# duongve13112002/DiffusionSpatialControl

Hardware: AMD Instinct MI355X
Metric: 512x512 images/sec, SD1.5 25-step DPM++2M Karras with region-biased cross-attention (higher is better)
Workload: dtype f16; 1 GPU; SD1.5 512x512, 25-step DPM++2M Karras, CFG 7.5, 2 region masks, 1 image(s) per generation, 2 generation(s) in flight per GPU; images_per_gpu=1, parallelism=dp1 (independent images, no per-step collective), hip_graph=True, outputs_finite=True, full=False

## Files before the change

diffusionspatialcontrol_amd/_lib.py:

```python
import ctypes
import os
import re

_HERE = os.path.dirname(os.path.abspath(__file__))
_LIB = None


class DscLibraryError(RuntimeError):
    pass


def lib_path():
    return os.environ.get("DSC_LIB_PATH") or os.path.join(_HERE, "libdsc_hip.so")


def header_path():
    return os.path.join(os.path.dirname(_HERE), "include", "dsc_hip.h")


def declared_symbols():
    txt = open(header_path()).read()
    txt = re.sub(r"/\*.*?\*/", "", txt, flags=re.S)
    return sorted(set(re.findall(r"\b(dsc_[a-z0-9_]+)\s*\(", txt)))

# ... 75 lines not shown
                                          ctypes.c_int, ctypes.c_int, _vp, ctypes.c_int, _vp, ctypes.c_float, ctypes.c_int, _vp]),
    "dsc_add_layernorm": (ctypes.c_int, [_vp] * 6 + [ctypes.c_int64, ctypes.c_int, ctypes.c_float, ctypes.c_int, _vp]),
    "dsc_geglu": (ctypes.c_int, [_vp, _vp, ctypes.c_int64, ctypes.c_int, ctypes.c_int, _vp]),
    "dsc_linear_splitk_workspace_bytes": (ctypes.c_size_t, [ctypes.c_int64, ctypes.c_int, ctypes.c_int, ctypes.c_int]),
    "dsc_linear_splitk_f16": (ctypes.c_int, [_vp] * 5 + [ctypes.c_int64, ctypes.c_int, ctypes.c_int] + [ctypes.c_int64] * 3 +
                              [ctypes.c_int, _vp, ctypes.c_size_t, ctypes.c_int, _vp]),
    "dsc_conv3x3_gn_rows": (ctypes.c_int, [ctypes.c_int] * 7),
    "dsc_conv3x3_gn_nhwc_f16": (ctypes.c_int, [_vp] * 4 + [ctypes.c_int64, _vp, _vp] + [ctypes.c_int] * 5 + [ctypes.c_int64] * 3 +
                                [ctypes.c_int, _vp, ctypes.c_int, ctypes.c_int, _vp]),
    "dsc_linear_gn_rows": (ctypes.c_int, [ctypes.c_int64, ctypes.c_int, ctypes.c_int, ctypes.c_int, ctypes.c_int]),
    "dsc_linear_gn_f16": (ctypes.c_int, [_vp] * 5 + [ctypes.c_int64, ctypes.c_int, ctypes.c_int] + [ctypes.c_int64] * 3 +
                          [ctypes.c_int, _vp, ctypes.c_int, ctypes.c_int, _vp]),
    "dsc_groupnorm_apply_nhwc": (ctypes.c_int, [_vp] * 5 + [ctypes.c_int] * 5 + [ctypes.c_float, ctypes.c_int, ctypes.c_int, _vp]),
    "dsc_softmax_rows_f16": (ctypes.c_int, [_vp, _vp, ctypes.c_int64, ctypes.c_int, ctypes.c_int64, ctypes.c_int64, ctypes.c_float,
                                            ctypes.c_int, _vp]),
    "dsc_latent_resample_noise": (ctypes.c_int, [_vp] * 3 + [ctypes.c_int] * 6 + [_vp] * 4 + [ctypes.c_float, _vp]),
}


def load_library():
    global _LIB
    if _LIB is not None:
        return _LIB
    import torch
    path = lib_path()
    if not os.path.exists(path):
        raise DscLibraryError(
            f"{path} not found: build it with `python -c 'import __graft_entry__ as g; g.build()'` "
            "(hipcc --offload-arch=gfx950).  There is no CPU fallback for the HIP hot path.")
    try:
# ... 33 lines not shown
```

diffusionspatialcontrol_amd/csrc/conv3x3.hip:

```cpp
#include "dsc_common.h"
#include "dsc_hip.h"
#include "gn_partials.h"
#include <type_traits>

extern int g_dsc_tuning_profile;

namespace {

constexpr int BM = 128, BN = 64, BK = 64, T = 256;
constexpr int kBStageBytes = BN * BK * 2;
constexpr int kAPiecesMax = 25;
constexpr int kABytes = kAPiecesMax * 1024;
constexpr int kRingOff = 0;
constexpr int a_off(int S) { return S * kBStageBytes; }
constexpr int pad_off(int S) { return a_off(S) + 2 * kABytes; }
constexpr int lds_bytes(int S) { return pad_off(S) + 1024; }
constexpr int a_bytes(int NT, int TW) { return NT == 4 && TW == 16 ? 23 * 1024 : kABytes; }
constexpr int lds_bytes_up2x(int TW) { return a_off(4) + 2 * a_bytes(4, TW) + 1024; }
constexpr int kEpiStride = BN + 4;
constexpr unsigned kOob = 0x80000000u;

struct ConvParams {
    const half_t* x; const half_t* w; const half_t* bias; const half_t* res; half_t* out; float* ws;
    int B, H, W, Cin, Cout;
// ... 485 lines not shown
        9ll * Cin * Cout >= (1ll << 30)) return 0;
    return plan(B, H, W, Cin, Cout, 0, &p) ? 1 : 0;
}

extern "C" size_t dsc_conv3x3_workspace_bytes(int B, int H, int W, int Cin, int Cout, int splits) {
    ConvParams p{};
    if (B <= 0 || H <= 0 || W <= 0 || !plan(B, H, W, Cin, Cout, splits, &p)) return 0;
    return p.splits > 1 ? (size_t)p.splits * p.npix * Cout * sizeof(float) : 0;
}

namespace {
struct GnArgs { const void* add; int64_t add_ld; float* part; int groups; };
int conv_impl(const void* x, const void* w, const void* bias, const void* residual, void* out,
              int B, int H, int W, int Cin, int Cout, int64_t ldx, int64_t ldr, int64_t ldo,
              int resample, int out_nchw, int splits, int dtype, void* workspace, size_t workspace_bytes, void* stream,
              const GnArgs* gn);
}

extern "C" int dsc_conv3x3_nhwc_f16(const void* x, const void* w, const void* bias, const void* residual, void* out,
                                    int B, int H, int W, int Cin, int Cout, int64_t ldx, int64_t ldr, int64_t ldo,
                                    int resample, int out_nchw, int splits, int dtype, void* workspace,
                                    size_t workspace_bytes, void* stream) {
    return conv_impl(x, w, bias, residual, out, B, H, W, Cin, Cout, ldx, ldr, ldo, resample, out_nchw, splits, dtype, workspace,
                     workspace_bytes, stream, nullptr);
}

extern "C" int dsc_conv3x3_gn_rows(int B, int H, int W, int Cin, int Cout, int groups, int resample) {
    ConvParams p{};
    const int Hc = H, Wc = W;
    if (B <= 0 || H <= 0 || W <= 0 || groups <= 0 || Cout % BN != 0 || Cout % groups != 0 || Cout / groups > 64 || Cout / groups < 2) return 0;
    if (resample == DSC_CONV_STRIDE2 || resample == DSC_CONV_STRIDE2_PAD_BR) return 0;
// ... 5 lines not shown
extern "C" int dsc_conv3x3_gn_nhwc_f16(const void* x, const void* w, const void* bias, const void* add, int64_t add_ld,
                                       const void* residual, void* out, int B, int H, int W, int Cin, int Cout, int64_t ldx,
                                       int64_t ldr, int64_t ldo, int resample, float* gn_part, int groups, int dtype, void* stream) {
    if (!gn_part || groups <= 0) return DSC_ERR_BAD_ARG;
    if (!dsc_conv3x3_gn_rows(B, H, W, Cin, Cout, groups, resample)) return DSC_ERR_UNSUPPORTED;
    if (add && (add_ld < Cout || add_ld % 8 != 0 || (reinterpret_cast<uintptr_t>(add) & 15))) return DSC_ERR_UNSUPPORTED;
    if (reinterpret_cast<uintptr_t>(gn_part) & 7) return DSC_ERR_UNSUPPORTED;
    const GnArgs gn{add, add_ld, gn_part, groups};
    return conv_impl(x, w, bias, residual, out, B, H, W, Cin, Cout, ldx, ldr, ldo, resample, 0, 1, dtype, nullptr, 0, stream, &gn);
}

namespace {
int conv_impl(const void* x, const void* w, const void* bias, const void* residual, void* out,
              int B, int H, int W, int Cin, int Cout, int64_t ldx, int64_t ldr, int64_t ldo,
              int resample, int out_nchw, int splits, int dtype, void* workspace, size_t workspace_bytes, void* stream,
              const GnArgs* gn) {
    if (!x || !w || !out || B <= 0 || H <= 0 || W <= 0 || Cin <= 0 || Cout <= 0) return DSC_ERR_BAD_ARG;
    if (dtype != DSC_F16) return DSC_ERR_UNSUPPORTED;
    if (ldx < Cin || (!out_nchw && ldo < Cout) || (residual && ldr < Cout)) return DSC_ERR_BAD_ARG;
    if (ldx % 8 != 0 || (Cout % 8 == 0 && !out_nchw && ldo % 8 != 0) || (residual && Cout % 8 == 0 && ldr % 8 != 0)) return DSC_ERR_UNSUPPORTED;
    if (!al16(x) || !al16(w) || !al16(out) || (bias && !al16(bias)) || (residual && !al16(residual))) return DSC_ERR_UNSUPPORTED;
    if ((long long)B * H * W * (ldx > ldo ? ldx : ldo) >= (1ll << 30) || 9ll * Cin * Cout >= (1ll << 30)) return DSC_ERR_UNSUPPORTED;
    ConvParams p{};
    const int tw = plan(B, H, W, Cin, Cout, splits, &p);
    if (!tw) return DSC_ERR_UNSUPPORTED;
    p.x = static_cast<const half_t*>(x); p.w = static_cast<const half_t*>(w);
    p.bias = static_cast<const half_t*>(bias); p.res = static_cast<const half_t*>(residual);
    p.out = static_cast<half_t*>(out); p.ws = static_cast<float*>(workspace);
    p.ldx = ldx; p.ldr = ldr; p.ldo = ldo;
    p.stamps = g_conv_stamps;
    if (gn) {
        p.add = static_cast<const half_t*>(gn->add); p.add_ld = gn->add_ld;
        p.gn_part = gn->part; p.gn_G = gn->groups; p.gn_cpg = Cout / gn->groups;
    }
    p.order = g_conv_order >= 0 ? g_conv_order : (p.npix >= 2ll * Cout ? 1 : 0);
    if (resample < 0 || resample > 4 || ((resample == DSC_CONV_STRIDE2 || resample == DSC_CONV_STRIDE2_PAD_BR) && out_nchw)) return DSC_ERR_UNSUPPORTED;
    if (resample == DSC_CONV_STRIDE2_PAD_BR && ((H | W) & 1)) return DSC_ERR_UNSUPPORTED;
    p.up = resample == DSC_CONV_UPSAMPLE2X || resample == DSC_CONV_UPSAMPLE_CEIL ? 1 : 0;
    p.sh = resample == DSC_CONV_UPSAMPLE_CEIL ? (H + 1) / 2 : H / 2; p.sw = resample == DSC_CONV_UPSAMPLE_CEIL ? (W + 1) / 2 : W / 2;
    p.sub2 = resample == DSC_CONV_STRIDE2 ? 1 : (resample == DSC_CONV_STRIDE2_PAD_BR ? 2 : 0);
// ... 22 lines not shown
    const dim3 grid(((total + 7) / 8) * 8), block(T);
    int ring = g_conv_ring;
    if (ring != 3 && ring != 9) ring = (total <= 256 && g_dsc_tuning_profile == DSC_TUNE_LATENCY) ? 9 : 3;
    const bool loaders = ring == 9 && (g_conv_loaders == 2 || (g_conv_loaders == 1 && tw == 16));
    const dim3 block8(T + 256);
    if (tw == 16) {
        if (loaders) DSC_LAUNCH((conv3x3_kernel<16, 9, 4>), grid, block8, (size_t)lds_bytes(9), st, p);
        else if (ring == 9) DSC_LAUNCH((conv3x3_kernel<16, 9>), grid, block, (size_t)lds_bytes(9), st, p);
        else DSC_LAUNCH((conv3x3_kernel<16, 3>), grid, block, (size_t)lds_bytes(3), st, p);
    } else {
        if (loaders) DSC_LAUNCH((conv3x3_kernel<8, 9, 4>), grid, block8, (size_t)lds_bytes(9), st, p);
        else if (ring == 9) DSC_LAUNCH((conv3x3_kernel<8, 9>), grid, block, (size_t)lds_bytes(9), st, p);
        else DSC_LAUNCH((conv3x3_kernel<8, 3>), grid, block, (size_t)lds_bytes(3), st, p);
    }
    if (hipGetLastError() != hipSuccess) return DSC_ERR_LAUNCH;
    if (p.splits > 1) {
        const long long n = p.onpix * (Cout / 8);
        p.fd_cv = make_fastdiv(Cout / 8, n + 256);
        DSC_LAUNCH(conv3x3_reduce, dim3((unsigned)((n + 255) / 256)), dim3(256), 0, st, p);
        if (hipGetLastError() != hipSuccess) return DSC_ERR_LAUNCH;
    }
    return DSC_OK;
}
}


namespace {

__global__ __launch_bounds__(256) void conv3x3_up2x_pack_kernel(const half_t* __restrict__ w, half_t* __restrict__ packed, int Cin, int Cout) {
    const int cv = Cin >> 3;
    const long long idx = (long long)blockIdx.x * 256 + threadIdx.x;
    if (idx >= 16ll * Cout * cv) return;
    const int c = (int)(idx % cv) * 8;
    const int tap = (int)(idx / cv) & 3;
    const long long pn = idx / cv / 4;
    const int n = (int)(pn % Cout), phase = (int)(pn / Cout);
    const int py = phase >> 1, px = phase & 1, a = tap >> 1, b = tap & 1;
    const int dy0 = py + a == 0 ? 0 : (py + a == 2 ? 2 : 1 - py), dy1 = py + a == 1 ? dy0 + 1 : dy0;
// ... 87 lines not shown
```

diffusionspatialcontrol_amd/csrc/gemm.hip:

```cpp
#include "dsc_common.h"
#include "dsc_hip.h"
#include "gn_partials.h"

extern int g_dsc_tuning_profile;

namespace {

constexpr int BN = 64, BK = 64, T = 256;
constexpr int kBHalves = BN * BK;
constexpr int a_halves(int bm) { return bm * BK; }
constexpr int stage_halves(int bm, int nt = 1) { return bm * BK + nt * kBHalves; }
constexpr int epi_stride(int nt = 1) { return nt * BN + 4; }
constexpr int kEpiStride = epi_stride(1);

struct GemmParams {
    const half_t* x; const half_t* w; const half_t* bias; const half_t* res; half_t* out;
    int M, N, K;
    long long ldx, ldr, ldo;
    const float* ln_in;
    const float* ln_c;
    float* ln_out;
    int ln_nb; float ln_inv_c, ln_eps;
    half_t* kv; int kv_C, kv_H, kv_d, kv_L, kv_B;
    int xcd_remap, total;
// ... 322 lines not shown
    const long long m = fdiv(idx, fd_cv);
    const int n = (idx - (int)m * cv) * 8;
    float acc[8] = {0, 0, 0, 0, 0, 0, 0, 0};
    for (int k = 0; k < splits; ++k) {
        const float* src = ws + ((long long)k * M + m) * N + n;
        const f4x_t a = *reinterpret_cast<const f4x_t*>(src), b = *reinterpret_cast<const f4x_t*>(src + 4);
#pragma unroll
        for (int j = 0; j < 4; ++j) { acc[j] += a[j]; acc[4 + j] += b[j]; }
    }
    h8_t bv = {0, 0, 0, 0, 0, 0, 0, 0}, rv = {0, 0, 0, 0, 0, 0, 0, 0};
    if (bias) bv = *reinterpret_cast<const h8_t*>(bias + n);
    if (res) rv = *reinterpret_cast<const h8_t*>(res + m * ldr + n);
    h8_t o;
#pragma unroll
    for (int j = 0; j < 8; ++j) o[j] = (half_t)(acc[j] + (float)bv[j] + (float)rv[j]);
    *reinterpret_cast<h8_t*>(out + m * ldo + n) = o;
}

bool al16(const void* q) { return (reinterpret_cast<uintptr_t>(q) & 15) == 0; }

long long* g_gemm_stamps = nullptr;
int g_gemm_stages = 0;
int g_gemm_bm = 0;
int g_gemm_loaders = 0;
int g_gemm_xcd = 0;
int g_gemm_wide_min = 512;
int g_gemm_ntstore = 0;
int g_gemm_nt = 0;

}
// ... 213 lines not shown
    if (splits <= 1) return dsc_linear_f16(x, w, bias, residual, out, M, N, K, ldx, ldr, ldo, 0, dtype, stream);
    if (residual && (ldr >> 32) != 0) return DSC_ERR_UNSUPPORTED;
    const size_t need = (size_t)splits * M * N * sizeof(float);
    if (!workspace || workspace_bytes < need || !al16(workspace)) return DSC_ERR_WORKSPACE;
    if ((bias && !al16(bias)) || (residual && (!al16(residual) || ldr % 8 != 0)) || ldo % 8 != 0 || !al16(out)) return DSC_ERR_UNSUPPORTED;
    const int rc = linear_impl(x, w, nullptr, nullptr, out, M, N, K, ldx, 0, ldo, 0, nullptr, 0, nullptr, 0.f, nullptr, dtype, stream,
                               nullptr, 0, 0, splits, static_cast<float*>(workspace));
    if (rc != DSC_OK) return rc;
    const long long n8 = M * (N / 8);
    if (n8 >= (1ll << 30)) return DSC_ERR_UNSUPPORTED;
    DSC_LAUNCH(gemm_splitk_reduce, dim3((unsigned)((n8 + 255) / 256)), dim3(256), 0, static_cast<hipStream_t>(stream),
               static_cast<const float*>(workspace), static_cast<const half_t*>(bias), static_cast<const half_t*>(residual),
               static_cast<half_t*>(out), (long long)M, N, splits, (long long)ldr, (long long)ldo, make_fastdiv(N / 8, n8 + 256));
    return hipGetLastError() == hipSuccess ? DSC_OK : DSC_ERR_LAUNCH;
}
```

diffusionspatialcontrol_amd/csrc/groupnorm_nhwc.hip:

```cpp
#include "dsc_common.h"
#include "dsc_hip.h"

namespace {

constexpr int kMaxT = 512;

struct GnN {
    const half_t* x; half_t* y; const half_t* gamma; const half_t* beta; const half_t* add;
    double* partials;
    float* stats;
    int B, HW, C, G, cpg, cv, k, nchunk, rows;
    int anchunk, arows;
    int inline_stats;
    int scv, nslab, sk;
    long long add_stride;
    float eps; int silu;
    const half_t* x2; half_t* cat; int C1;
    const float* fpart; int fPT;
    FastDiv fd_G, fd_anchunk, fd_cv, fd_cpg, fd_vpp, fd_nslab, fd_nchunk, fd_scv;
};

__device__ __forceinline__ h8_t gn_load(const GnN& p, int b, int pix, int c) {
    const long long bp = (long long)b * p.HW + pix;
    if (!p.x2) return *reinterpret_cast<const h8_t*>(p.x + bp * p.C + c);
    const h8_t v = c < p.C1 ? *reinterpret_cast<const h8_t*>(p.x + bp * p.C1 + c)
                            : *reinterpret_cast<const h8_t*>(p.x2 + bp * (p.C - p.C1) + (c - p.C1));
    *reinterpret_cast<h8_t*>(p.cat + bp * p.C + c) = v;
    return v;
}

__global__ __launch_bounds__(kMaxT) void gn_nhwc_stats(GnN p) {
    extern __shared__ __attribute__((aligned(16))) char smem[];
    const int bc = fdiv(blockIdx.x, p.fd_nslab), slab = blockIdx.x - bc * p.nslab;
    const int b = fdiv(bc, p.fd_nchunk), chunk = bc - b * p.nchunk;
    const int v0 = slab * p.scv;
// ... 232 lines not shown
    for (int i = 0; i < kSmallVec; ++i) {
        const int idx = threadIdx.x + 256 * i;
        if (idx < nvec) {
            const int pix = fdiv(idx, p.fd_vpp), j8 = idx - pix * vpp;
            const h8_t ga = gav[i], be = bev[i];
            h8_t o;
#pragma unroll
            for (int j = 0; j < 8; ++j) {
                float f = (v[i][j] - mean) * rstd * (float)ga[j] + (float)be[j];
                if (p.silu) f = silu_f(f);
                o[j] = (half_t)f;
            }
            *reinterpret_cast<h8_t*>(p.y + base + (long long)pix * p.C + j8 * 8) = o;
        }
    }
}

struct GnBundle { int gb, nvec, npl; };

template <int T, int NV>
__global__ __launch_bounds__(T) void gn_nhwc_bundle(GnN p, GnBundle q) {
    extern __shared__ __attribute__((aligned(16))) char smem[];
    float* S = reinterpret_cast<float*>(smem);
    __shared__ float gstat[8];
    const int nb = p.G / q.gb;
    const int b = blockIdx.x / nb, bun = blockIdx.x % nb;
    const int cw = q.nvec * 8;
    const int t = threadIdx.x;
    const bool active = t < q.nvec * q.npl;
    const int v = t % q.nvec, lp = t / q.nvec;
// ... 280 lines not shown
                                        void* stream) {
    if (!x || !y || !gamma || !beta || !gn_part || part_rows <= 0 || B <= 0 || C <= 0 || hw <= 0 || groups <= 0) return DSC_ERR_BAD_ARG;
    if (dtype != DSC_F16) return DSC_ERR_UNSUPPORTED;
    GnN p{};
    p.B = B; p.C = C; p.HW = hw; p.G = groups;
    if (!plan(p) || p.cpg > 64 || C % 64 != 0) return DSC_ERR_UNSUPPORTED;
    if (!al16(x) || !al16(y) || !al16(gamma) || !al16(beta) || !al16(gn_part)) return DSC_ERR_UNSUPPORTED;
    p.x = static_cast<const half_t*>(x); p.y = static_cast<half_t*>(y);
    p.gamma = static_cast<const half_t*>(gamma); p.beta = static_cast<const half_t*>(beta);
    p.eps = eps; p.silu = apply_silu;
    p.fpart = gn_part; p.fPT = part_rows; p.inline_stats = 1;
    gn_fastdivs(p);
    DSC_LAUNCH(gn_nhwc_apply, dim3(B * p.anchunk), dim3(p.cv * p.k), 0, static_cast<hipStream_t>(stream), p);
    return hipGetLastError() == hipSuccess ? DSC_OK : DSC_ERR_LAUNCH;
}
```

diffusionspatialcontrol_amd/modules/u_net_condition_modify.py:

```python
import inspect
import math
from dataclasses import dataclass, field
from typing import Any, Dict, Optional, Tuple

import torch
import torch.nn as nn
import torch.nn.functional as F

from .. import ops
from .attention_modify import AttnProcessor, AttnProcessor2_0


class ImageProjection(nn.Module):

    def __init__(self, image_embed_dim=768, cross_attention_dim=768, num_image_text_embeds=32):
        super().__init__()
        self.num_image_text_embeds = num_image_text_embeds
        self.image_embeds = nn.Linear(image_embed_dim, num_image_text_embeds * cross_attention_dim)
        self.norm = nn.LayerNorm(cross_attention_dim)

    def forward(self, image_embeds):
        b = image_embeds.shape[0]
        return self.norm(self.image_embeds(image_embeds).reshape(b, self.num_image_text_embeds, -1))

# ... 460 lines not shown
        return _derived(self, "tb", (self.time_emb_proj.bias, self.conv1.bias),
                        lambda: (self.time_emb_proj.bias + self.conv1.bias).contiguous())

    def forward(self, x, temb_act, temb_add=None):
        if isinstance(x, tuple):
            h, x = self.norm1.of_cat(*x)
        else:
            h = self.norm1(x)
        if temb_add is None:
            temb_add = F.linear(temb_act, self.time_emb_proj.weight, self.temb_bias())
        g = self.norm2.num_groups
        fuse = h.is_cuda and h.dtype == torch.float16 and h.shape[0] * h.shape[2] * h.shape[3] >= GN_FUSE_MIN_ROWS
        if fuse and ops.conv3x3_gn_rows(h, self.conv1.weight, g) > 0:
            h = self.norm2(ops.conv3x3_gn(h, self.conv1.weight, g, add=temb_add[:h.shape[0]]))
        else:
            h = self.norm2(_conv3x3(h, self.conv1.weight), add=temb_add)
        if self.conv_shortcut is None:
            if fuse and ops.conv3x3_gn_rows(h, self.conv2.weight, g) > 0:
                return ops.conv3x3_gn(h, self.conv2.weight, g, bias=self.conv2.bias, residual=x)
            return _conv3x3(h, self.conv2.weight, self.conv2.bias, residual=x)
        h = _conv3x3(h, self.conv2.weight)
        b = _derived(self, "sb", (self.conv_shortcut.bias, self.conv2.bias),
                     lambda: (self.conv_shortcut.bias + self.conv2.bias).contiguous())
        bsz, _, hh, ww = h.shape
        t, part = self.conv_shortcut.tokens(_tokens(x), bias=b, residual=_tokens(h), gn_groups=g)
        return _with_gn(_image(t, hh, ww), part)


class Downsample2D(nn.Module):
    def __init__(self, c):
        super().__init__()
        self.conv = nn.Conv2d(c, c, 3, stride=2, padding=1)

    def forward(self, x):
        if ops.conv3x3_supported(x, self.conv.weight):
            return ops.conv3x3(x, self.conv.weight, self.conv.bias, stride2_ceil=True)
        return self.conv(x)


# ... 301 lines not shown
```

diffusionspatialcontrol_amd/ops.py:

```python
import ctypes
import os

import numpy as np
import torch

from . import _lib

FLAG_REF_FP16_ROUNDING = 1
FLAG_BIAS_IS_FINAL = 2
FLAG_REUSE_STATS = 4
FLAG_ROWS_PADDED = 256
FLAG_SIGMA_PER_GROUP = 512
REGION_ROW_STRIDE = 100

def _stream_ptr(t):
    return ctypes.c_void_p(torch.cuda.current_stream(t.device).cuda_stream)


def _p(t):
    return ctypes.c_void_p(t.data_ptr()) if t is not None else None


def _i64x3(a, b, c):
    return (ctypes.c_int64 * 3)(a, b, c)
# ... 572 lines not shown
        part, cvec, eps = ln
        nb = part.shape[1]
        if part.shape[0] != M or part.dtype != torch.float32 or not part.is_contiguous() or cvec.numel() != 3 * C:
            raise ValueError("linear_qkv: statistics / cvec do not match the operands")
    rc = _lib.load_library().dsc_linear_qkv_f16(_p(x2), _p(weight), _p(bias), _p(q), _p(kv), M, C, K, x2.stride(0), C, heads, L,
                                                _p(part), nb, _p(cvec), float(eps), 0, _stream_ptr(x))
    _lib.check(rc, "dsc_linear_qkv_f16")
    return q.view(B, L, heads, d), kv[0].permute(0, 2, 1, 3), kv[1].permute(0, 2, 1, 3)


USE_SPLITK = os.environ.get("DSC_GEMM_SPLITK", "1") != "0"
SPLITK_MAX_ROWS = int(os.environ.get("DSC_SPLITK_MAX_ROWS", "512"))
SPLITK_MIN_K = int(os.environ.get("DSC_SPLITK_MIN_K", "1920"))


def linear_splitk(x2, weight, bias, r2, splits=0):
    lib = _lib.load_library()
    M, K = x2.shape
    N = weight.shape[0]
    out = torch.empty((M, N), dtype=x2.dtype, device=x2.device)
    nbytes = lib.dsc_linear_splitk_workspace_bytes(M, N, K, splits)
    ws = _workspace(x2.device, nbytes) if nbytes else None
    rc = lib.dsc_linear_splitk_f16(_p(x2), _p(weight), _p(bias), _p(r2), _p(out), M, N, K, x2.stride(0),
                                   r2.stride(0) if r2 is not None else 0, N, splits, _p(ws), ws.numel() * 8 if ws is not None else 0,
                                   0, _stream_ptr(x2))
    _lib.check(rc, "dsc_linear_splitk_f16")
    return out


def linear(x, weight, bias=None, residual=None, geglu=False, prefer_kernel=False):
# ... 9 lines not shown
    x2 = None
    if can:
        x2 = x.reshape(M, K)
        can = x2.stride(1) == 1 and x2.stride(0) % 8 == 0 and x2.data_ptr() % 16 == 0
    ldr = 0
    if residual is not None and residual.numel() != M * N:
        got = _residual_2d(residual, M, N) if can and not geglu else None
        if got is None or not (prefer_kernel or _gemm_rows_k_preferred(M, K, geglu)):
            residual = residual.reshape(-1, N).repeat(M // (residual.numel() // N), 1).reshape(*lead, N)
    if can and residual is not None:
        got = _residual_2d(residual, M, N)
        can = got is not None
        if can:
            r2, ldr = got
    ok = can and (prefer_kernel or _gemm_rows_k_preferred(M, K, geglu))
    if can and not ok and not geglu and USE_SPLITK and not USE_LIBRARY_GEMM and M <= SPLITK_MAX_ROWS and K >= SPLITK_MIN_K \
            and (bias is None or (bias.dtype == torch.float16 and bias.data_ptr() % 16 == 0)):
        return linear_splitk(x2, weight, bias, residual.reshape(M, N) if residual is not None else None).reshape(*lead, N)
    if not ok:
        if ((USE_LT_RESIDUAL if residual is not None else USE_LT_ALL) and x.dtype == torch.float16 and K % 8 == 0
                and N % 8 == 0 and M >= 8 and not (geglu and residual is not None)):
            xl = x.reshape(M, K)
            rl = residual.reshape(M, N) if residual is not None else None
            if (xl.stride(1) == 1 and xl.stride(0) % 8 == 0 and weight.is_contiguous() and weight.dtype == torch.float16
                    and (bias is None or bias.dtype == torch.float16)
                    and (rl is None or (rl.stride(1) == 1 and rl.stride(0) % 8 == 0))):
                out = torch.empty((M, N), dtype=x.dtype, device=x.device)
                rc = _lib.load_library().dsc_linear_lt_f16(_p(xl), _p(weight), _p(bias), _p(rl), _p(out), M, N, K,
                                                           xl.stride(0), rl.stride(0) if rl is not None else 0, N, 0,
                                                           _stream_ptr(x))
                if rc == 0:
                    out = out.reshape(*lead, N)
# ... 70 lines not shown
        out = torch.empty((B, Cout, oh, ow), dtype=x.dtype, device=x.device, memory_format=cl)
    ldr = 0
    if residual is not None:
        if residual.shape != out.shape:
            raise ValueError("conv3x3: residual must have the output's shape")
        if not residual.is_contiguous(memory_format=cl):
            residual = residual.contiguous(memory_format=cl)
        ldr = Cout
    nbytes = lib.dsc_conv3x3_workspace_bytes(B, H, W, Cin, Cout, splits)
    ws = _workspace(x.device, nbytes) if nbytes else None
    rc = lib.dsc_conv3x3_nhwc_f16(_p(x), _p(weight), _p(bias), _p(residual), _p(out), B, H, W, Cin, Cout, Cin, ldr, Cout,
                                  3 if stride2_pad_br else (2 if stride2 else (1 if upsample else (4 if size is not None else 0))), 1 if out_nchw else 0, splits, 0, _p(ws),
                                  ws.numel() * 8 if ws is not None else 0, _stream_ptr(x))
    _lib.check(rc, "dsc_conv3x3_nhwc_f16")
    return out


USE_UP2X_PHASES = os.environ.get("DSC_UP2X_PHASES", "1") != "0"


def conv3x3_up2x_pack(weight):
    _require_gpu(weight)
    if weight.dim() != 4 or tuple(weight.shape[2:]) != (3, 3) or weight.dtype != torch.float16:
        raise ValueError("conv3x3_up2x_pack: weight must be a [Cout, Cin, 3, 3] fp16 tensor")
    Cout, Cin = weight.shape[:2]
    if Cin % 64 != 0:
        raise ValueError("conv3x3_up2x_pack: Cin must be a multiple of 64")
    cl = torch.channels_last
    if not weight.is_contiguous(memory_format=cl):
        weight = weight.contiguous(memory_format=cl)
# ... 340 lines not shown
```

include/dsc_hip.h:

```cpp
#ifndef DSC_HIP_H
#define DSC_HIP_H

#include <stddef.h>
#include <stdint.h>

#ifdef __cplusplus
extern "C" {
#endif

#define DSC_OK                0
#define DSC_ERR_BAD_ARG      -1
#define DSC_ERR_UNSUPPORTED  -2
#define DSC_ERR_WORKSPACE    -3
#define DSC_ERR_LAUNCH       -4

#define DSC_F16 0
#define DSC_FLAG_REF_FP16_ROUNDING 1u
#define DSC_FLAG_REUSE_STATS       4u
#define DSC_FLAG_ROWS_PADDED     256u
#define DSC_FLAG_BIAS_IS_FINAL     2u
#define DSC_FLAG_SIGMA_PER_GROUP 512u

int dsc_abi_version(void);
const char* dsc_target_arch(void);
// ... 95 lines not shown
size_t dsc_groupnorm_workspace_bytes(int B, int C, int hw, int groups);
int dsc_groupnorm_silu(const void* x, void* y, const void* gamma, const void* beta,
                       int B, int C, int hw, int groups, float eps, int apply_silu, int dtype,
                       void* workspace, size_t workspace_bytes, void* stream);

size_t dsc_groupnorm_nhwc_workspace_bytes(int B, int C, int hw, int groups);
void dsc_debug_set_gn_mode(int mode);
int dsc_groupnorm_silu_nhwc(const void* x, void* y, const void* gamma, const void* beta,
                            const void* add, int64_t add_row_stride,
                            int B, int C, int hw, int groups, float eps, int apply_silu, int dtype,
                            void* workspace, size_t workspace_bytes, void* stream);
int dsc_groupnorm_silu_nhwc_cat(const void* x1, const void* x2, int C1, void* cat, void* y, const void* gamma,
                                const void* beta, const void* add, int64_t add_row_stride, int B, int C, int hw,
                                int groups, float eps, int apply_silu, int dtype, void* workspace, size_t workspace_bytes,
                                void* stream);

int dsc_add_bias_residual(const void* a, const void* b, const void* bias, void* out, int64_t rows, int C,
                          int dtype, void* stream);

int dsc_linear_f16(const void* x, const void* w, const void* bias, const void* residual, void* out,
                   int64_t M, int N, int K, int64_t ldx, int64_t ldr, int64_t ldo, int geglu, int dtype, void* stream);

#define DSC_CONV_UPSAMPLE2X 1
#define DSC_CONV_STRIDE2 2
#define DSC_CONV_STRIDE2_PAD_BR 3
#define DSC_CONV_UPSAMPLE_CEIL 4
int dsc_conv3x3_supported(int B, int H, int W, int Cin, int Cout);
void dsc_debug_set_conv_stamps(void* device_buffer);
void dsc_debug_set_conv_ring(int stages);
size_t dsc_conv3x3_workspace_bytes(int B, int H, int W, int Cin, int Cout, int splits);
int dsc_conv3x3_nhwc_f16(const void* x, const void* w, const void* bias, const void* residual, void* out,
                         int B, int H, int W, int Cin, int Cout, int64_t ldx, int64_t ldr, int64_t ldo,
                         int resample, int out_nchw, int splits, int dtype, void* workspace, size_t workspace_bytes,
                         void* stream);

int dsc_conv3x3_up2x_pack_f16(const void* w, void* packed, int Cin, int Cout, void* stream);
int dsc_conv3x3_up2x_supported(int B, int h, int w, int Cin, int Cout);
size_t dsc_conv3x3_up2x_workspace_bytes(int B, int h, int w, int Cin, int Cout, int splits);
int dsc_conv3x3_up2x_nhwc_f16(const void* x, const void* w_packed, const void* bias, void* out, int B, int h, int w,
                              int Cin, int Cout, int splits, void* workspace, size_t workspace_bytes, int64_t ldx,
                              int64_t ldo, int dtype, void* stream);

int dsc_linear_ln_f16(const void* x, const void* w, const void* bias, const void* residual, void* out,
                      int64_t M, int N, int K, int64_t ldx, int64_t ldr, int64_t ldo, int geglu,
                      const float* ln_in, int ln_nb, const float* ln_cvec, float ln_eps, float* ln_out,
                      int dtype, void* stream);
void dsc_debug_set_gemm_stages(int stages);
int dsc_linear_qkv_f16(const void* x, const void* w, const void* bias, void* q_out, void* kv_out,
                       int64_t M, int C, int K, int64_t ldx, int64_t ldq, int heads, int seq_len,
// ... 26 lines not shown
int dsc_conv3x3_gn_nhwc_f16(const void* x, const void* w, const void* bias, const void* add, int64_t add_ld,
                            const void* residual, void* out, int B, int H, int W, int Cin, int Cout, int64_t ldx,
                            int64_t ldr, int64_t ldo, int resample, float* gn_part, int groups, int dtype, void* stream);
int dsc_linear_gn_rows(int64_t M, int N, int K, int rows_per_image, int groups);
int dsc_linear_gn_f16(const void* x, const void* w, const void* bias, const void* residual, void* out,
                      int64_t M, int N, int K, int64_t ldx, int64_t ldr, int64_t ldo, int rows_per_image,
                      float* gn_part, int groups, int dtype, void* stream);
int dsc_groupnorm_apply_nhwc(const void* x, void* y, const void* gamma, const void* beta, const float* gn_part,
                             int part_rows, int B, int C, int hw, int groups, float eps, int apply_silu, int dtype,
                             void* stream);

size_t dsc_linear_splitk_workspace_bytes(int64_t M, int N, int K, int splits);
int dsc_linear_splitk_f16(const void* x, const void* w, const void* bias, const void* residual, void* out,
                          int64_t M, int N, int K, int64_t ldx, int64_t ldr, int64_t ldo, int splits,
                          void* workspace, size_t workspace_bytes, int dtype, void* stream);

int dsc_softmax_rows_f16(const void* scores, void* probs, int64_t rows, int n, int64_t ld_scores, int64_t ld_probs,
                         float scale, int dtype, void* stream);

int dsc_latent_resample_noise(const void* src, const void* noise, void* dst, int n, int C, int h, int w, int H, int W,
                              const int* idx_y, const float* w_y, const int* idx_x, const float* w_x,
                              float noise_scale_f16_value, void* stream);

#ifdef __cplusplus
}
#endif
#endif
```

Baseline: 11.90 images/s.

## Fold split-K conv partial-plane reduction into groupnorm and shortcut GEMM reduce

For small-resolution ResNet blocks where the 3x3 conv runs split-K, a new path skips the separate conv reduce kernel. The fp32 partial planes are summed directly inside the consumer: either a new groupnorm+SiLU kernel or the shortcut linear's split-K reduce. This removes one kernel launch and an f16 round trip of the conv output per affected layer. In exchange the consumer kernels read S fp32 planes, and the new path replicates the f16 rounding of the intermediate.

```diff
diff --git a/diffusionspatialcontrol_amd/_lib.py b/diffusionspatialcontrol_amd/_lib.py
--- a/diffusionspatialcontrol_amd/_lib.py
+++ b/diffusionspatialcontrol_amd/_lib.py
@@ -113,6 +113,15 @@
     "dsc_groupnorm_apply_nhwc": (ctypes.c_int, [_vp] * 5 + [ctypes.c_int] * 5 + [ctypes.c_float, ctypes.c_int, ctypes.c_int, _vp]),
     "dsc_softmax_rows_f16": (ctypes.c_int, [_vp, _vp, ctypes.c_int64, ctypes.c_int, ctypes.c_int64, ctypes.c_int64, ctypes.c_float,
                                             ctypes.c_int, _vp]),
+    "dsc_conv3x3_splits": (ctypes.c_int, [ctypes.c_int] * 6),
+    "dsc_conv3x3_planes_f16": (ctypes.c_int, [_vp, _vp] + [ctypes.c_int] * 5 + [ctypes.c_int64, ctypes.c_int, ctypes.c_int, _vp,
+                                                                               ctypes.c_size_t, _vp]),
+    "dsc_groupnorm_nhwc_planes_covers": (ctypes.c_int, [ctypes.c_int] * 4),
+    "dsc_groupnorm_silu_nhwc_planes": (ctypes.c_int, [_vp, ctypes.c_int, ctypes.c_size_t, _vp, _vp, ctypes.c_int64] + [_vp] * 4 +
+                                       [ctypes.c_int64] + [ctypes.c_int] * 4 + [ctypes.c_float, ctypes.c_int, ctypes.c_int, _vp]),
+    "dsc_linear_splitk_planes_f16": (ctypes.c_int, [_vp] * 4 + [ctypes.c_int, ctypes.c_size_t, _vp, ctypes.c_int64, ctypes.c_int,
+                                                            ctypes.c_int, ctypes.c_int64, ctypes.c_int64, ctypes.c_int, _vp,
+                                                            ctypes.c_size_t, ctypes.c_int, _vp]),
     "dsc_latent_resample_noise": (ctypes.c_int, [_vp] * 3 + [ctypes.c_int] * 6 + [_vp] * 4 + [ctypes.c_float, _vp]),
 }
 
diff --git a/diffusionspatialcontrol_amd/csrc/conv3x3.hip b/diffusionspatialcontrol_amd/csrc/conv3x3.hip
--- a/diffusionspatialcontrol_amd/csrc/conv3x3.hip
+++ b/diffusionspatialcontrol_amd/csrc/conv3x3.hip
@@ -523,7 +523,7 @@
 int conv_impl(const void* x, const void* w, const void* bias, const void* residual, void* out,
               int B, int H, int W, int Cin, int Cout, int64_t ldx, int64_t ldr, int64_t ldo,
               int resample, int out_nchw, int splits, int dtype, void* workspace, size_t workspace_bytes, void* stream,
-              const GnArgs* gn);
+              const GnArgs* gn, bool planes_only = false);
 }
 
 extern "C" int dsc_conv3x3_nhwc_f16(const void* x, const void* w, const void* bias, const void* residual, void* out,
@@ -559,16 +559,17 @@
 int conv_impl(const void* x, const void* w, const void* bias, const void* residual, void* out,
               int B, int H, int W, int Cin, int Cout, int64_t ldx, int64_t ldr, int64_t ldo,
               int resample, int out_nchw, int splits, int dtype, void* workspace, size_t workspace_bytes, void* stream,
-              const GnArgs* gn) {
-    if (!x || !w || !out || B <= 0 || H <= 0 || W <= 0 || Cin <= 0 || Cout <= 0) return DSC_ERR_BAD_ARG;
+              const GnArgs* gn, bool planes_only) {
+    if (!x || !w || (!out && !planes_only) || B <= 0 || H <= 0 || W <= 0 || Cin <= 0 || Cout <= 0) return DSC_ERR_BAD_ARG;
     if (dtype != DSC_F16) return DSC_ERR_UNSUPPORTED;
     if (ldx < Cin || (!out_nchw && ldo < Cout) || (residual && ldr < Cout)) return DSC_ERR_BAD_ARG;
     if (ldx % 8 != 0 || (Cout % 8 == 0 && !out_nchw && ldo % 8 != 0) || (residual && Cout % 8 == 0 && ldr % 8 != 0)) return DSC_ERR_UNSUPPORTED;
-    if (!al16(x) || !al16(w) || !al16(out) || (bias && !al16(bias)) || (residual && !al16(residual))) return DSC_ERR_UNSUPPORTED;
+    if (!al16(x) || !al16(w) || (!planes_only && !al16(out)) || (bias && !al16(bias)) || (residual && !al16(residual))) return DSC_ERR_UNSUPPORTED;
     if ((long long)B * H * W * (ldx > ldo ? ldx : ldo) >= (1ll << 30) || 9ll * Cin * Cout >= (1ll << 30)) return DSC_ERR_UNSUPPORTED;
     ConvParams p{};
     const int tw = plan(B, H, W, Cin, Cout, splits, &p);
     if (!tw) return DSC_ERR_UNSUPPORTED;
+    if (planes_only && p.splits < 2) return DSC_ERR_UNSUPPORTED;
     p.x = static_cast<const half_t*>(x); p.w = static_cast<const half_t*>(w);
     p.bias = static_cast<const half_t*>(bias); p.res = static_cast<const half_t*>(residual);
     p.out = static_cast<half_t*>(out); p.ws = static_cast<float*>(workspace);
@@ -621,7 +622,7 @@
         else DSC_LAUNCH((conv3x3_kernel<8, 3>), grid, block, (size_t)lds_bytes(3), st, p);
     }
     if (hipGetLastError() != hipSuccess) return DSC_ERR_LAUNCH;
-    if (p.splits > 1) {
+    if (p.splits > 1 && !planes_only) {
         const long long n = p.onpix * (Cout / 8);
         p.fd_cv = make_fastdiv(Cout / 8, n + 256);
         DSC_LAUNCH(conv3x3_reduce, dim3((unsigned)((n + 255) / 256)), dim3(256), 0, st, p);
@@ -629,6 +630,19 @@
     }
     return DSC_OK;
 }
+}
+
+extern "C" int dsc_conv3x3_splits(int B, int H, int W, int Cin, int Cout, int splits) {
+    ConvParams p{};
+    if (!dsc_conv3x3_supported(B, H, W, Cin, Cout) || !plan(B, H, W, Cin, Cout, splits, &p)) return 0;
+    return p.splits;
+}
+
+extern "C" int dsc_conv3x3_planes_f16(const void* x, const void* w, int B, int H, int W, int Cin, int Cout, int64_t ldx, int splits,
+                                      int dtype, void* planes, size_t planes_bytes, void* stream) {
+    if (!planes) return DSC_ERR_BAD_ARG;
+    return conv_impl(x, w, nullptr, nullptr, nullptr, B, H, W, Cin, Cout, ldx, 0, Cout, 0, 0, splits, dtype, planes, planes_bytes,
+                     stream, nullptr, true);
 }
 
 
diff --git a/diffusionspatialcontrol_amd/csrc/gemm.hip b/diffusionspatialcontrol_amd/csrc/gemm.hip
--- a/diffusionspatialcontrol_amd/csrc/gemm.hip
+++ b/diffusionspatialcontrol_amd/csrc/gemm.hip
@@ -360,6 +360,37 @@
     h8_t o;
 #pragma unroll
     for (int j = 0; j < 8; ++j) o[j] = (half_t)(acc[j] + (float)bv[j] + (float)rv[j]);
+    *reinterpret_cast<h8_t*>(out + m * ldo + n) = o;
+}
+
+__global__ __launch_bounds__(256) void gemm_splitk_reduce_planes(const float* ws, const half_t* bias, const float* rp, int Sr, half_t* out,
+                                                                 long long M, int N, int splits, long long ldo, FastDiv fd_cv) {
+    const int cv = N >> 3;
+    const int idx = blockIdx.x * 256 + threadIdx.x;
+    if (idx >= (int)M * cv) return;
+    const long long m = fdiv(idx, fd_cv);
+    const int n = (idx - (int)m * cv) * 8;
+    float r[8] = {0, 0, 0, 0, 0, 0, 0, 0}, acc[8] = {0, 0, 0, 0, 0, 0, 0, 0};
+    for (int k = 0; k < Sr; ++k) {
+        const float* src = rp + ((long long)k * M + m) * N + n;
+        const f4x_t a = *reinterpret_cast<const f4x_t*>(src), b = *reinterpret_cast<const f4x_t*>(src + 4);
+#pragma unroll
+        for (int j = 0; j < 4; ++j) { r[j] += a[j]; r[4 + j] += b[j]; }
+    }
+    for (int k = 0; k < splits; ++k) {
+        const float* src = ws + ((long long)k * M + m) * N + n;
+        const f4x_t a = *reinterpret_cast<const f4x_t*>(src), b = *reinterpret_cast<const f4x_t*>(src + 4);
+#pragma unroll
+        for (int j = 0; j < 4; ++j) { acc[j] += a[j]; acc[4 + j] += b[j]; }
+    }
+    h8_t bv = {0, 0, 0, 0, 0, 0, 0, 0};
+    if (bias) bv = *reinterpret_cast<const h8_t*>(bias + n);
+    h8_t o;
+#pragma unroll
+    for (int j = 0; j < 8; ++j) {
+        const half_t rv = (half_t)(r[j] + 0.f + 0.f);
+        o[j] = (half_t)(acc[j] + (float)bv[j] + (float)rv);
+    }
     *reinterpret_cast<h8_t*>(out + m * ldo + n) = o;
 }
 
@@ -603,3 +634,27 @@
                static_cast<half_t*>(out), (long long)M, N, splits, (long long)ldr, (long long)ldo, make_fastdiv(N / 8, n8 + 256));
     return hipGetLastError() == hipSuccess ? DSC_OK : DSC_ERR_LAUNCH;
 }
+
+extern "C" int dsc_linear_splitk_planes_f16(const void* x, const void* w, const void* bias, const void* rplanes, int Sr,
+                                            size_t rplanes_bytes, void* out, int64_t M, int N, int K, int64_t ldx, int64_t ldo,
+                                            int splits, void* workspace, size_t workspace_bytes, int dtype, void* stream) {
+    if (!x || !w || !out || !rplanes || M <= 0 || N <= 0 || K <= 0 || Sr < 2) return DSC_ERR_BAD_ARG;
+    if (dtype != DSC_F16 || K % BK != 0 || N % BN != 0) return DSC_ERR_UNSUPPORTED;
+    if (splits <= 0) splits = splitk_auto(M, N, K);
+    const int nkt = K / BK, kps = (nkt + splits - 1) / splits;
+    splits = (nkt + kps - 1) / kps;
+    if (splits <= 1) return DSC_ERR_UNSUPPORTED;
+    const size_t need = (size_t)splits * M * N * sizeof(float);
+    if (!workspace || workspace_bytes < need || !al16(workspace)) return DSC_ERR_WORKSPACE;
+    if (rplanes_bytes < (size_t)Sr * M * N * sizeof(float)) return DSC_ERR_WORKSPACE;
+    if ((bias && !al16(bias)) || !al16(rplanes) || ldo % 8 != 0 || !al16(out)) return DSC_ERR_UNSUPPORTED;
+    const long long n8 = M * (N / 8);
+    if (n8 >= (1ll << 30)) return DSC_ERR_UNSUPPORTED;
+    const int rc = linear_impl(x, w, nullptr, nullptr, out, M, N, K, ldx, 0, ldo, 0, nullptr, 0, nullptr, 0.f, nullptr, dtype, stream,
+                               nullptr, 0, 0, splits, static_cast<float*>(workspace));
+    if (rc != DSC_OK) return rc;
+    DSC_LAUNCH(gemm_splitk_reduce_planes, dim3((unsigned)((n8 + 255) / 256)), dim3(256), 0, static_cast<hipStream_t>(stream),
+               static_cast<const float*>(workspace), static_cast<const half_t*>(bias), static_cast<const float*>(rplanes), Sr,
+               static_cast<half_t*>(out), (long long)M, N, splits, (long long)ldo, make_fastdiv(N / 8, n8 + 256));
+    return hipGetLastError() == hipSuccess ? DSC_OK : DSC_ERR_LAUNCH;
+}
diff --git a/diffusionspatialcontrol_amd/csrc/groupnorm_nhwc.hip b/diffusionspatialcontrol_amd/csrc/groupnorm_nhwc.hip
--- a/diffusionspatialcontrol_amd/csrc/groupnorm_nhwc.hip
+++ b/diffusionspatialcontrol_amd/csrc/groupnorm_nhwc.hip
@@ -19,6 +19,8 @@
     const float* fpart; int fPT;
     FastDiv fd_G, fd_anchunk, fd_cv, fd_cpg, fd_vpp, fd_nslab, fd_nchunk, fd_scv;
 };
+
+struct GnPlanes { const float* planes; int S; const half_t* bias; const half_t* res; long long ldr; };
 
 __device__ __forceinline__ h8_t gn_load(const GnN& p, int b, int pix, int c) {
     const long long bp = (long long)b * p.HW + pix;
@@ -281,6 +283,119 @@
             *reinterpret_cast<h8_t*>(p.y + base + (long long)pix * p.C + j8 * 8) = o;
         }
     }
+}
+
+template <int NV>
+__device__ __forceinline__ void gn_small_finish(const GnN& p, const float (&v)[NV][8], const h8_t (&gav)[NV], const h8_t (&bev)[NV],
+                                                float s1, float* red, int vpp, int nvec, long long base) {
+    const int lane = threadIdx.x & 63, wave = threadIdx.x >> 6;
+    s1 = wave_sum_f32(s1);
+    if (lane == 0) red[wave] = s1;
+    __syncthreads();
+    const float n = (float)p.HW * p.cpg;
+    const float mean = (red[0] + red[1] + red[2] + red[3]) / n;
+    float s2 = 0.f;
+#pragma unroll
+    for (int i = 0; i < NV; ++i) {
+        const int idx = threadIdx.x + 256 * i;
+        if (idx < nvec) {
+#pragma unroll
+            for (int j = 0; j < 8; ++j) { const float dlt = v[i][j] - mean; s2 += dlt * dlt; }
+        }
+    }
+    s2 = wave_sum_f32(s2);
+    if (lane == 0) red[4 + wave] = s2;
+    __syncthreads();
+    const float rstd = rsqrtf((red[4] + red[5] + red[6] + red[7]) / n + p.eps);
+#pragma unroll
+    for (int i = 0; i < NV; ++i) {
+        const int idx = threadIdx.x + 256 * i;
+        if (idx < nvec) {
+            const int pix = fdiv(idx, p.fd_vpp), j8 = idx - pix * vpp;
+            const h8_t ga = gav[i], be = bev[i];
+            h8_t o;
+#pragma unroll
+            for (int j = 0; j < 8; ++j) {
+                float f = (v[i][j] - mean) * rstd * (float)ga[j] + (float)be[j];
+                if (p.silu) f = silu_f(f);
+                o[j] = (half_t)f;
+            }
+            *reinterpret_cast<h8_t*>(p.y + base + (long long)pix * p.C + j8 * 8) = o;
+        }
+    }
+}
+
+template <int NV, int KU>
+__global__ __launch_bounds__(256) void gn_nhwc_small_planes(GnN p, GnPlanes q) {
+    __shared__ float red[8];
+    const int b = fdiv(blockIdx.x, p.fd_G), g = blockIdx.x - b * p.G;
+    const int vpp = p.cpg >> 3;
+    const int nvec = p.HW * vpp;
+    const long long base = (long long)b * p.HW * p.C + g * p.cpg;
+    const long long pstride = (long long)p.B * p.HW * p.C;
+    float v[NV][8];
+    h8_t adv[NV];
+    int off[NV];
+#pragma unroll
+    for (int i = 0; i < NV; ++i) {
+        const int idx = threadIdx.x + 256 * i;
+        off[i] = -1;
+        adv[i] = h8_t{0, 0, 0, 0, 0, 0, 0, 0};
+        if (idx < nvec) {
+            const int pix = fdiv(idx, p.fd_vpp), j8 = idx - pix * vpp;
+            off[i] = (int)base + pix * p.C + j8 * 8;
+            if (p.add) adv[i] = *reinterpret_cast<const h8_t*>(p.add + (long long)b * p.add_stride + g * p.cpg + j8 * 8);
+        }
+#pragma unroll
+        for (int j = 0; j < 8; ++j) v[i][j] = 0.f;
+    }
+    for (int k0 = 0; k0 < q.S; k0 += KU) {
+        f4x_t a[KU][NV][2];
+#pragma unroll
+        for (int u = 0; u < KU; ++u)
+#pragma unroll
+            for (int i = 0; i < NV; ++i) {
+                a[u][i][0] = f4x_t{0.f, 0.f, 0.f, 0.f}; a[u][i][1] = a[u][i][0];
+                if (off[i] >= 0 && k0 + u < q.S) {
+                    const float* src = q.planes + (long long)(k0 + u) * pstride + off[i];
+                    a[u][i][0] = *reinterpret_cast<const f4x_t*>(src); a[u][i][1] = *reinterpret_cast<const f4x_t*>(src + 4);
+                }
+            }
+#pragma unroll
+        for (int u = 0; u < KU; ++u)
+#pragma unroll
+            for (int i = 0; i < NV; ++i)
+                if (off[i] >= 0 && k0 + u < q.S) {
+#pragma unroll
+                    for (int j = 0; j < 4; ++j) { v[i][j] += a[u][i][0][j]; v[i][4 + j] += a[u][i][1][j]; }
+                }
+    }
+    h8_t gav[NV], bev[NV], bv[NV], rv[NV];
+#pragma unroll
+    for (int i = 0; i < NV; ++i) {
+        const int idx = threadIdx.x + 256 * i;
+        gav[i] = h8_t{0, 0, 0, 0, 0, 0, 0, 0}; bev[i] = gav[i]; bv[i] = gav[i]; rv[i] = gav[i];
+        if (idx < nvec) {
+            const int pix = fdiv(idx, p.fd_vpp), c = g * p.cpg + (idx - pix * vpp) * 8;
+            if (q.bias) bv[i] = *reinterpret_cast<const h8_t*>(q.bias + c);
+            if (q.res) rv[i] = *reinterpret_cast<const h8_t*>(q.res + ((long long)b * p.HW + pix) * q.ldr + c);
+            gav[i] = *reinterpret_cast<const h8_t*>(p.gamma + c);
+            bev[i] = *reinterpret_cast<const h8_t*>(p.beta + c);
+        }
+    }
+    float s1 = 0.f;
+#pragma unroll
+    for (int i = 0; i < NV; ++i) {
+        if (off[i] >= 0) {
+#pragma unroll
+            for (int j = 0; j < 8; ++j) {
+                const half_t x = (half_t)(v[i][j] + (float)bv[i][j] + (float)rv[i][j]);
+                v[i][j] = (float)x + (float)adv[i][j];
+                s1 += v[i][j];
+            }
+        }
+    }
+    gn_small_finish<NV>(p, v, gav, bev, s1, red, vpp, nvec, base);
 }
 
 struct GnBundle { int gb, nvec, npl; };
@@ -591,3 +706,39 @@
     DSC_LAUNCH(gn_nhwc_apply, dim3(B * p.anchunk), dim3(p.cv * p.k), 0, static_cast<hipStream_t>(stream), p);
     return hipGetLastError() == hipSuccess ? DSC_OK : DSC_ERR_LAUNCH;
 }
+
+extern "C" int dsc_groupnorm_nhwc_planes_covers(int B, int C, int hw, int groups) {
+    GnN p{};
+    p.B = B; p.C = C; p.HW = hw; p.G = groups;
+    if (B <= 0 || C <= 0 || hw <= 0 || groups <= 0 || !plan(p) || g_gn_mode == 2) return 0;
+    if ((long long)B * hw * C >= (1ll << 30)) return 0;
+    return p.cpg % 8 == 0 && (long long)hw * (p.cpg / 8) <= 256 * kSmallVec ? 1 : 0;
+}
+
+extern "C" int dsc_groupnorm_silu_nhwc_planes(const void* planes, int S, size_t planes_bytes, const void* bias, const void* residual,
+                                              int64_t ldr, void* y, const void* gamma, const void* beta, const void* add,
+                                              int64_t add_row_stride, int B, int C, int hw, int groups, float eps, int apply_silu,
+                                              int dtype, void* stream) {
+    if (!planes || !y || !gamma || !beta || B <= 0 || C <= 0 || hw <= 0 || groups <= 0) return DSC_ERR_BAD_ARG;
+    if (S < 2) return DSC_ERR_BAD_ARG;
+    if (dtype != DSC_F16) return DSC_ERR_UNSUPPORTED;
+    if (!dsc_groupnorm_nhwc_planes_covers(B, C, hw, groups)) return DSC_ERR_UNSUPPORTED;
+    if (!al16(planes) || !al16(y) || !al16(gamma) || !al16(beta) || (bias && !al16(bias)) ||
+        (residual && (!al16(residual) || ldr % 8 != 0 || ldr < C)) ||
+        (add && (!al16(add) || add_row_stride % 8 != 0 || add_row_stride < C)))
+        return DSC_ERR_UNSUPPORTED;
+    if (planes_bytes < (size_t)S * B * hw * C * sizeof(float)) return DSC_ERR_WORKSPACE;
+    GnN p{};
+    p.B = B; p.C = C; p.HW = hw; p.G = groups;
+    plan(p);
+    p.y = static_cast<half_t*>(y);
+    p.gamma = static_cast<const half_t*>(gamma); p.beta = static_cast<const half_t*>(beta);
+    p.add = static_cast<const half_t*>(add); p.add_stride = add_row_stride;
+    const GnPlanes q{static_cast<const float*>(planes), S, static_cast<const half_t*>(bias), static_cast<const half_t*>(residual), ldr};
+    p.eps = eps; p.silu = apply_silu;
+    gn_fastdivs(p);
+    hipStream_t st = static_cast<hipStream_t>(stream);
+    if ((long long)hw * (p.cpg / 8) <= 256 * 2) DSC_LAUNCH((gn_nhwc_small_planes<2, 5>), dim3(B * groups), dim3(256), 0, st, p, q);
+    else DSC_LAUNCH((gn_nhwc_small_planes<kSmallVec, 2>), dim3(B * groups), dim3(256), 0, st, p, q);
+    return hipGetLastError() == hipSuccess ? DSC_OK : DSC_ERR_LAUNCH;
+}
diff --git a/diffusionspatialcontrol_amd/modules/u_net_condition_modify.py b/diffusionspatialcontrol_amd/modules/u_net_condition_modify.py
--- a/diffusionspatialcontrol_amd/modules/u_net_condition_modify.py
+++ b/diffusionspatialcontrol_amd/modules/u_net_condition_modify.py
@@ -498,15 +498,28 @@
         if fuse and ops.conv3x3_gn_rows(h, self.conv1.weight, g) > 0:
             h = self.norm2(ops.conv3x3_gn(h, self.conv1.weight, g, add=temb_add[:h.shape[0]]))
         else:
-            h = self.norm2(_conv3x3(h, self.conv1.weight), add=temb_add)
+            n2, cout = self.norm2, self.conv1.weight.shape[0]
+            planes = None
+            if ops.USE_SUM_FOLD and h.is_cuda and ops.groupnorm_planes_covers(h.shape[0], cout, h.shape[2] * h.shape[3], g):
+                planes = ops.conv3x3_planes(h, self.conv1.weight)
+            if planes is not None:
+                h = ops.groupnorm_silu_nhwc_planes(*planes, (h.shape[0], cout, h.shape[2], h.shape[3]), g, n2.weight, n2.bias,
+                                                   n2.eps, n2.act, add=temb_add)
+            else:
+                h = n2(_conv3x3(h, self.conv1.weight), add=temb_add)
         if self.conv_shortcut is None:
             if fuse and ops.conv3x3_gn_rows(h, self.conv2.weight, g) > 0:
                 return ops.conv3x3_gn(h, self.conv2.weight, g, bias=self.conv2.bias, residual=x)
             return _conv3x3(h, self.conv2.weight, self.conv2.bias, residual=x)
-        h = _conv3x3(h, self.conv2.weight)
         b = _derived(self, "sb", (self.conv_shortcut.bias, self.conv2.bias),
                      lambda: (self.conv_shortcut.bias + self.conv2.bias).contiguous())
         bsz, _, hh, ww = h.shape
+        if ops.USE_SUM_FOLD and h.is_cuda and bsz * hh * ww < GN_FUSE_MIN_ROWS:
+            xt, ws = _tokens(x), self.conv_shortcut.weight.flatten(1)
+            planes = ops.conv3x3_planes(h, self.conv2.weight) if ops.linear_splitk_covers(xt, ws, b) else None
+            if planes is not None:
+                return _with_gn(_image(ops.linear_splitk_planes(xt, ws, b, *planes), hh, ww), None)
+        h = _conv3x3(h, self.conv2.weight)
         t, part = self.conv_shortcut.tokens(_tokens(x), bias=b, residual=_tokens(h), gn_groups=g)
         return _with_gn(_image(t, hh, ww), part)
 
diff --git a/diffusionspatialcontrol_amd/ops.py b/diffusionspatialcontrol_amd/ops.py
--- a/diffusionspatialcontrol_amd/ops.py
+++ b/diffusionspatialcontrol_amd/ops.py
@@ -610,6 +610,11 @@
 SPLITK_MIN_K = int(os.environ.get("DSC_SPLITK_MIN_K", "1920"))
 
 
+def _splitk_route(M, K, geglu, bias):
+    return (not geglu and USE_SPLITK and not USE_LIBRARY_GEMM and M <= SPLITK_MAX_ROWS and K >= SPLITK_MIN_K
+            and (bias is None or (bias.dtype == torch.float16 and bias.data_ptr() % 16 == 0)))
+
+
 def linear_splitk(x2, weight, bias, r2, splits=0):
     lib = _lib.load_library()
     M, K = x2.shape
@@ -649,8 +654,7 @@
         if can:
             r2, ldr = got
     ok = can and (prefer_kernel or _gemm_rows_k_preferred(M, K, geglu))
-    if can and not ok and not geglu and USE_SPLITK and not USE_LIBRARY_GEMM and M <= SPLITK_MAX_ROWS and K >= SPLITK_MIN_K \
-            and (bias is None or (bias.dtype == torch.float16 and bias.data_ptr() % 16 == 0)):
+    if can and not ok and _splitk_route(M, K, geglu, bias):
         return linear_splitk(x2, weight, bias, residual.reshape(M, N) if residual is not None else None).reshape(*lead, N)
     if not ok:
         if ((USE_LT_RESIDUAL if residual is not None else USE_LT_ALL) and x.dtype == torch.float16 and K % 8 == 0
@@ -751,6 +755,84 @@
                                   ws.numel() * 8 if ws is not None else 0, _stream_ptr(x))
     _lib.check(rc, "dsc_conv3x3_nhwc_f16")
     return out
+
+
+USE_SUM_FOLD = os.environ.get("DSC_SUM_FOLD", "1") != "0"
+SUM_FOLD_COUNTS = {"groupnorm": 0, "shortcut": 0}
+
+
+def conv3x3_splits(x, weight, splits=0):
+    if not conv3x3_supported(x, weight):
+        return 0
+    B, Cin, H, W = x.shape
+    return int(_lib.load_library().dsc_conv3x3_splits(B, H, W, Cin, weight.shape[0], splits))
+
+
+def conv3x3_planes(x, weight, splits=0):
+    S = conv3x3_splits(x, weight, splits)
+    if S < 2:
+        return None
+    lib = _lib.load_library()
+    cl = torch.channels_last
+    if not x.is_contiguous(memory_format=cl):
+        x = x.contiguous(memory_format=cl)
+    if not weight.is_contiguous(memory_format=cl):
+        weight = weight.contiguous(memory_format=cl)
+    B, Cin, H, W = x.shape
+    Cout = weight.shape[0]
+    planes = _workspace(x.device, lib.dsc_conv3x3_workspace_bytes(B, H, W, Cin, Cout, splits))
+    rc = lib.dsc_conv3x3_planes_f16(_p(x), _p(weight), B, H, W, Cin, Cout, Cin, splits, 0, _p(planes), planes.numel() * 8,
+                                    _stream_ptr(x))
+    _lib.check(rc, "dsc_conv3x3_planes_f16")
+    return planes, S
+
+
+def groupnorm_planes_covers(B, C, hw, groups):
+    return bool(_lib.load_library().dsc_groupnorm_nhwc_planes_covers(B, C, hw, groups))
+
+
+def groupnorm_silu_nhwc_planes(planes, S, shape, groups, weight, bias, eps, act, add=None, conv_bias=None, residual=None):
+    B, C, h, w = shape
+    y = torch.empty((B, C, h, w), dtype=torch.float16, device=planes.device, memory_format=torch.channels_last)
+    add_stride = 0
+    if add is not None:
+        if add.stride(-1) != 1 or add.stride(0) % 8 != 0 or add.data_ptr() % 16 != 0:
+            add = add.contiguous()
+        add_stride = add.stride(0)
+    if residual is not None:
+        if tuple(residual.shape) != (B, C, h, w):
+            raise ValueError("groupnorm_silu_nhwc_planes: residual must have the convolution output's shape")
+        if not residual.is_contiguous(memory_format=torch.channels_last):
+            residual = residual.contiguous(memory_format=torch.channels_last)
+    rc = _lib.load_library().dsc_groupnorm_silu_nhwc_planes(
+        _p(planes), S, planes.numel() * 8, _p(conv_bias), _p(residual), C if residual is not None else 0, _p(y), _p(weight),
+        _p(bias), _p(add), add_stride, B, C, h * w, groups, float(eps), 1 if act else 0, 0, _stream_ptr(planes))
+    _lib.check(rc, "dsc_groupnorm_silu_nhwc_planes")
+    SUM_FOLD_COUNTS["groupnorm"] += 1
+    return y
+
+
+def linear_splitk_covers(x, weight, bias):
+    N, K = weight.shape
+    M = x.numel() // K
+    if not (USE_DSC_GEMM and x.is_cuda and linear_kernel_can(x, weight, bias, None)) or _gemm_rows_k_preferred(M, K):
+        return False
+    return _splitk_route(M, K, False, bias) and _lib.load_library().dsc_linear_splitk_workspace_bytes(M, N, K, 0) > 0
+
+
+def linear_splitk_planes(x, weight, bias, planes, S, splits=0):
+    lib = _lib.load_library()
+    N, K = weight.shape
+    lead = x.shape[:-1]
+    x2 = x.reshape(-1, K)
+    M = x2.shape[0]
+    out = torch.empty((M, N), dtype=x.dtype, device=x.device)
+    ws = _workspace(x.device, lib.dsc_linear_splitk_workspace_bytes(M, N, K, splits))
+    rc = lib.dsc_linear_splitk_planes_f16(_p(x2), _p(weight), _p(bias), _p(planes), S, planes.numel() * 8, _p(out), M, N, K,
+                                          x2.stride(0), N, splits, _p(ws), ws.numel() * 8, 0, _stream_ptr(x))
+    _lib.check(rc, "dsc_linear_splitk_planes_f16")
+    SUM_FOLD_COUNTS["shortcut"] += 1
+    return out.reshape(*lead, N)
 
 
 USE_UP2X_PHASES = os.environ.get("DSC_UP2X_PHASES", "1") != "0"
diff --git a/include/dsc_hip.h b/include/dsc_hip.h
--- a/include/dsc_hip.h
+++ b/include/dsc_hip.h
@@ -133,6 +133,11 @@
                                 const void* beta, const void* add, int64_t add_row_stride, int B, int C, int hw,
                                 int groups, float eps, int apply_silu, int dtype, void* workspace, size_t workspace_bytes,
                                 void* stream);
+int dsc_groupnorm_nhwc_planes_covers(int B, int C, int hw, int groups);
+int dsc_groupnorm_silu_nhwc_planes(const void* planes, int S, size_t planes_bytes, const void* bias, const void* residual,
+                                   int64_t ldr, void* y, const void* gamma, const void* beta, const void* add,
+                                   int64_t add_row_stride, int B, int C, int hw, int groups, float eps, int apply_silu,
+                                   int dtype, void* stream);
 
 int dsc_add_bias_residual(const void* a, const void* b, const void* bias, void* out, int64_t rows, int C,
                           int dtype, void* stream);
@@ -152,6 +157,9 @@
                          int B, int H, int W, int Cin, int Cout, int64_t ldx, int64_t ldr, int64_t ldo,
                          int resample, int out_nchw, int splits, int dtype, void* workspace, size_t workspace_bytes,
                          void* stream);
+int dsc_conv3x3_splits(int B, int H, int W, int Cin, int Cout, int splits);
+int dsc_conv3x3_planes_f16(const void* x, const void* w, int B, int H, int W, int Cin, int Cout, int64_t ldx, int splits,
+                           int dtype, void* planes, size_t planes_bytes, void* stream);
 
 int dsc_conv3x3_up2x_pack_f16(const void* w, void* packed, int Cin, int Cout, void* stream);
 int dsc_conv3x3_up2x_supported(int B, int h, int w, int Cin, int Cout);
@@ -208,6 +216,9 @@
 int dsc_linear_splitk_f16(const void* x, const void* w, const void* bias, const void* residual, void* out,
                           int64_t M, int N, int K, int64_t ldx, int64_t ldr, int64_t ldo, int splits,
                           void* workspace, size_t workspace_bytes, int dtype, void* stream);
+int dsc_linear_splitk_planes_f16(const void* x, const void* w, const void* bias, const void* rplanes, int Sr,
+                                 size_t rplanes_bytes, void* out, int64_t M, int N, int K, int64_t ldx, int64_t ldo, int splits,
+                                 void* workspace, size_t workspace_bytes, int dtype, void* stream);
 
 int dsc_softmax_rows_f16(const void* scores, void* probs, int64_t rows, int n, int64_t ld_scores, int64_t ld_probs,
                          float scale, int dtype, void* stream);
```

Result: no change. 11.86 images/s (-0.4%).
